# JinPLu/VeloxSeg

Measured on AMD Instinct MI355X. Metric: training patches/s on 128^3 2-mod volumes (fwd+loss+bwd+allreduce+AdamW), higher is better.
Workload: dtype f32

## Files before the change

include/veloxseg_hip.h:

```cpp
#ifndef VELOXSEG_HIP_H
#define VELOXSEG_HIP_H

#ifdef __cplusplus
extern "C" {
#endif

#define VX_ABI_VERSION 1

int vx_abi_version(void);
const char* vx_last_error(void);

int vx_conv3d_fwd(const float* x, const float* x2, int C1, const float* w, const float* bias, float* y,
                  int B, int Cin, int Di, int Hi, int Wi, int Cout, int K, int S, int P, int G, int ps, void* stream);
int vx_conv3d_bwd_data(const float* dy, const float* w, const float* bias_like, float* dx, float* dx2, int C1,
                       int B, int Cin, int Di, int Hi, int Wi, int Cout, int K, int S, int P, int G, int ps,
                       int accumulate, void* stream);
int vx_conv3d_bwd_weight(const float* x, const float* x2, int C1, const float* dy, float* dw, float* db,
                         int B, int Cin, int Di, int Hi, int Wi, int Cout, int K, int S, int P, int G, int ps, void* stream);

int vx_conv3d_bwd_weight_tiled(const float* x, const float* x2, int C1, const float* dy, float* dw, float* db,
                               int B, int Cin, int Di, int Hi, int Wi, int Cout, int K, int S, int P, int G, int ps, void* stream);
int vx_down_wgrad_ws_floats(int B, int Cin, int Di, int Hi, int Wi, int Cout);
int vx_down_wgrad_mfma(const float* x, const float* dy, float* dw, float* db, float* ws, long ws_floats,
                       int B, int Cin, int Di, int Hi, int Wi, int Cout, void* stream);
// ... 152 lines not shown
int vx_ln_cf_bwd(const float* x, const float* gamma, const float* dout, float* dx, float* dgamma, float* dbeta, float* ws,
                 int B, int C, long V, float eps, void* stream);
int vx_ln_cf_bwd_add(const float* x, const float* gamma, const float* dout, const float* add, float* dx, float* dgamma, float* dbeta, float* ws,
                     int B, int C, long V, float eps, void* stream);
int vx_ln_cf_bwd_data(const float* x, const float* gamma, const float* dout, const float* add, float* dx, float* ws, int B, int C, long V, float eps, void* stream);
int vx_ln_cf_bwd_param(const float* x, const float* dout, const float* ws, float* dgamma, float* dbeta, int B, int C, long V, void* stream);

int vx_gelu_drop_fwd(const float* a, float* h, long n, const void* seed_ptr, unsigned long long dstream, float p, void* stream);
int vx_gelu_drop_bwd(const float* dh, const float* a, float* da, long n, const void* seed_ptr, unsigned long long dstream, float p, void* stream);
int vx_axpy_drop_fwd(const float* x, const float* z, float* out, float alpha, long n, const void* seed_ptr, unsigned long long dstream, float p, void* stream);
int vx_axpy_drop_bwd(const float* dout, float* dx, float* dz, float alpha, long n, const void* seed_ptr, unsigned long long dstream, float p, void* stream);
int vx_add(const float* a, const float* b, const float* c, float* out, long n, void* stream);
int vx_add_many(const float* const* a, const float* const* b, const float* const* c, float* const* out, const long* n, int count, void* stream);
int vx_channel_sum(const float* dy, float* db, int B, int C, long V, void* stream);
int vx_space_to_depth2(const float* x, float* out, int B, int C, int Dc, int Hc, int Wc, int inverse, void* stream);
int vx_patchify(const float* x, float* out, int B, int C, int d, int h, int w, int K, void* stream);
int vx_patchify_bs(const float* x, long batch_stride, float* out, int B, int C, int d, int h, int w, int K, void* stream);
int vx_patchify_bs_h(const float* x, long batch_stride, void* out, int B, int C, int d, int h, int w, int K, int out_h16, void* stream);
int vx_patch_embed_ok(int Cin, int Cout, int Do, int Ho, int Wo, int K);
int vx_patch_embed_fwd(const float* x, long batch_stride, const float* w, const float* bias, float* y, int B, int Cin, int Cout, int Do, int Ho, int Wo, void* stream);
int vx_patch_embed_bwd_weight(const float* x, long batch_stride, const float* dy, float* dw, float* db, int B, int Cin, int Cout, int Do, int Ho, int Wo, void* stream);

typedef struct VxPwaPlan {
    int grid[3];
    int n[3];
    int heads, nb;
    int small[4][3];
    int nwin[4][3];
    int woff[4];
    int Ntot;
    int l;
} VxPwaPlan;

int vx_pwa_gather_fwd(const float* src, float* tok, const VxPwaPlan* plan, int c, int m, int M, int B, void* stream);
int vx_pwa_gather_bwd(const float* src, const float* dtok, float* dsrc, const VxPwaPlan* plan, int c, int m, int M, int B, void* stream);
int vx_pwa_gather_all_fwd(const float* const* srcs, float* tq, float* tk, float* tv, int* iq, int* ik, int* iv,
                          const VxPwaPlan* plan, int cq, int cv, int M, int B, void* stream);
int vx_pwa_gather_all_bwd(const float* dtq, const float* dtk, const float* dtv, const int* iq, const int* ik, const int* iv, float* const* dsrcs,
                          const VxPwaPlan* plan, int cq, int cv, int M, int B, void* stream);
int vx_pwa_scatter_fwd(const float* tok, float* out, const VxPwaPlan* plan, int c, int m, int M, int B, void* stream);
int vx_pwa_scatter_bwd(const float* dout, float* dtok, const VxPwaPlan* plan, int c, int m, int M, int B, void* stream);
int vx_pwa_scatter_fwd_all(const float* tok, float* const* outs, const VxPwaPlan* plan, int c, int M, int B, void* stream);
int vx_pwa_scatter_bwd_all(const float* const* douts, float* dtok, const VxPwaPlan* plan, int c, int M, int B, void* stream);
int vx_pwa_scatter_bwd_all_w(const float* const* douts, float* dtok, const VxPwaPlan* plan, int c, int M, int B, void* stream);
int vx_pwa_scatter_bwd_all_wz(const float* const* douts, float* dtok, const VxPwaPlan* plan, int c, int M, int B, float* extra_zero, long extra_floats, void* stream);
int vx_pwa_attn_set_fused_bwd(int on);
int vx_pwa_scatter_set_ident(int on);
int vx_pwa_attn_fwd(const float* Q, const float* K, const float* V, const float* table, float* O, float* LSE,
                    const VxPwaPlan* plan, int B, int M, int cq, int cv,
                    const void* seed_ptr, unsigned long long dstream, float p_drop, void* stream);
int vx_pwa_attn_bwd_ws_floats(const VxPwaPlan* plan, int B, int M);
int vx_pwa_attn_bwd_rep_offset(const VxPwaPlan* plan, int B, int M);
int vx_pwa_attn_bwd_mark_rep_zeroed(const float* delta_ws);
int vx_pwa_gather_set_vec(int on);
int vx_pwa_attn_bwd(const float* Q, const float* K, const float* V, const float* table, const float* O, const float* LSE,
                    const float* dO, float* dQ, float* dK, float* dV, float* dtable, float* delta_ws,
                    const VxPwaPlan* plan, int B, int M, int cq, int cv,
                    const void* seed_ptr, unsigned long long dstream, float p_drop, void* stream);
int vx_pwa_attn_bwd_nofold(const float* Q, const float* K, const float* V, const float* table, const float* O, const float* LSE,
                           const float* dO, float* dQ, float* dK, float* dV, float* delta_ws,
                           const VxPwaPlan* plan, int B, int M, int cq, int cv,
                           const void* seed_ptr, unsigned long long dstream, float p_drop, void* stream);
int vx_pwa_attn_bwd_fold(const float* delta_ws, float* dtable, const VxPwaPlan* plan, int B, int M, void* stream);
int vx_pwa_attn_bwd_fold_many(const float* const* delta_ws, float* const* dtables, const VxPwaPlan* const* plans, int count, int B, int M, void* stream);
int vx_pwa_attn_set_split(int S);
int vx_pwa_attn_bwd1_ok(const VxPwaPlan* plan, int B, int M, int cq, int cv);
int vx_pwa_attn_mbits_words(const VxPwaPlan* plan, int B, int M);
int vx_pwa_attn_mbits_useful(const VxPwaPlan* plan, int B, int M, int cq, int cv);
int vx_pwa_attn_set_valu_bits(int on);
int vx_pwa_attn_fwd_mb(const float* q, const float* k, const float* v, const float* table, float* out, float* lse, const VxPwaPlan* plan, int B, int M, int cq, int cv,
                       const void* seed_ptr, unsigned long long dstream, float p_drop, void* mbits, void* stream);
int vx_pwa_attn_bwd_mb(const float* q, const float* k, const float* v, const float* table, const float* out, const float* lse, const float* dout,
                       float* dq, float* dk, float* dv, float* dtable, float* delta_ws, const VxPwaPlan* plan, int B, int M, int cq, int cv,
                       const void* seed_ptr, unsigned long long dstream, float p_drop, const void* mbits, void* stream);
int vx_pwa_attn_bwd_nofold_mb(const float* q, const float* k, const float* v, const float* table, const float* out, const float* lse, const float* dout,
                              float* dq, float* dk, float* dv, float* delta_ws, const VxPwaPlan* plan, int B, int M, int cq, int cv,
                              const void* seed_ptr, unsigned long long dstream, float p_drop, const void* mbits, void* stream);
int vx_pwa_attn_mfma_ok(const VxPwaPlan* plan, int B, int M, int cq, int cv);
int vx_pwa_attn_set_mfma(int on);
int vx_pwa_attn_bwd1h_ok(const VxPwaPlan* plan, int B, int M, int cq, int cv);
int vx_pwa_attn_set_f16_bwd(int on);
int vx_pwa_attn_set_f16_bwd_ragged(int on);
int vx_pwa_attn_set_f16_bwd_m1(int on);
int vx_pwa_attn_set_short(int on);

int vx_seg_loss_fwd(const float* l0, const float* l1, const float* l2, const float* l3, int nh, const void* labels, int lab_kind,
                    double* acc, int B, int C, long V, void* stream);
int vx_sqdiff_sum(const float* a, const float* b, long n, double* acc, void* stream);
int vx_sqdiff_sum_bs(const float* a, const float* b, long n_per_sample, long b_batch_stride, int B, double* acc, void* stream);
int vx_mse_bwd_bs(const float* a, const float* b, long n_per_sample, long b_batch_stride, int B, const float* coef, const float* gout, float* da, void* stream);
int vx_sqdiff_sum_grad_bs(const float* a, const float* b, long n_per_sample, long b_batch_stride, int B, double* acc, float scale, float* da, void* stream);
int vx_sqdiff_sum_grad_bs_h(const void* a, const float* b, long n_per_sample, long b_batch_stride, int B, double* acc, float scale, void* da, int a_h16, void* stream);
int vx_loss_finalize(const double* seg_acc, int nh, int B, int C, long V, const float* head_weights,
                     const double* rc_acc, long n_rc, float w_rc,
                     const float* gram_seg, const float* g0, const float* g1, const float* g2, const float* g3, int M, int Cg, float w_f,
                     float* loss_out, float* coef, void* stream);
int vx_seg_loss_bwd(const float* logits, const void* labels, int lab_kind, const float* coef_head, const float* gout,
                    float* dlogits, int B, int C, long V, void* stream);
int vx_seg_loss_bwd4(const float* lg0, const float* lg1, const float* lg2, const float* lg3, int nh, const void* labels, int lab_kind, const float* coef,
                     int coef_stride, const float* gout, float* dl0, float* dl1, float* dl2, float* dl3, int B, int C, long V, void* stream);
int vx_seg_loss_ds_ok(int C, int D, int H, int W);
int vx_seg_loss_ds_set_columns(int on);
int vx_seg_loss_ds_ws_floats(const int* low_dims, int nh, int B, int C, int D);
int vx_seg_loss_ds_fwd(const float* l0, const float* l1, const float* l2, const float* l3, const int* low_dims, int nh, const void* labels, int lab_kind,
                       double* acc, int B, int C, int D, int H, int W, void* stream);
int vx_seg_loss_ds_bwd(const float* l0, const float* l1, const float* l2, const float* l3, const int* low_dims, int nh, const void* labels, int lab_kind,
                       const float* coef, int coef_stride, const float* gout, float* dl0, float* dl1, float* dl2, float* dl3, float* ws,
                       int B, int C, int D, int H, int W, void* stream);
int vx_seg_loss_ds_h16_ok(const int* low_dims, int nh, int B, int C, int D, int H, int W);
int vx_seg_loss_ds_fwd_h(const void* l0, const float* l1, const float* l2, const float* l3, const int* low_dims, int nh, const void* labels, int lab_kind,
                         double* acc, int B, int C, int D, int H, int W, int l0_h16, void* stream);
int vx_seg_loss_ds_bwd_h(const void* l0, const float* l1, const float* l2, const float* l3, const int* low_dims, int nh, const void* labels, int lab_kind,
                         const float* coef, int coef_stride, const float* gout, void* dl0, float* dl1, float* dl2, float* dl3, float* ws,
                         int B, int C, int D, int H, int W, int l0_h16, void* stream);
int vx_mse_bwd(const float* a, const float* b, const float* coef, const float* gout, float* da, long n, void* stream);
int vx_gram_mse_bwd(const float* gs, const float* g0, const float* g1, const float* g2, const float* g3, int M, const float* coef,
                    const float* gout, float* dgs, float* d0, float* d1, float* d2, float* d3, long n, void* stream);
int vx_gram_fwd(const float* x, float* G, int B, int C, long V, void* stream);
int vx_gram_bwd(const float* x, const float* dG, float* dx, int B, int C, long V, void* stream);
int vx_upsample_trilinear_fwd(const float* x, float* out, long BC, int d, int h, int w, int D, int H, int W, void* stream);
int vx_upsample_trilinear_bwd(const float* dout, float* dx, float* ws, long BC, int d, int h, int w, int D, int H, int W, void* stream);

int vx_upconv_set_mfma4(int on);
int vx_upconv_k2s2_fwd(const float* x, const float* w, const float* bias, float* y, int B, int Ci, int Co, int d, int h, int wd, void* stream);
int vx_upconv_k2s2_bwd_data(const float* dy, const float* w, float* dx, int B, int Ci, int Co, int d, int h, int wd, void* stream);
int vx_upconv_k2s2_wgrad_ok(int Ci, int Co);
int vx_upconv_k2s2_wgrad(const float* x, const float* dy, float* dw, int B, int Ci, int Co, int d, int h, int wd, void* stream);

int vx_adamw_step(float* p, const float* g, float* m, float* v, long n, float lr, float beta1, float beta2, float eps,
                  float weight_decay, long step, float grad_scale, void* stream);

int vx_sw_extract(const float* vol, float* win, int C, int D, int H, int W, int rd, int rh, int rw, int z0, int y0, int x0, void* stream);
int vx_sw_accumulate(const float* win, float* acc, int C, int D, int H, int W, int rd, int rh, int rw, int z0, int y0, int x0, float weight, void* stream);
int vx_sw_finalize(const float* acc, float* out, unsigned char* labels, const float* cz, const float* cy, const float* cx,
                   int C, int D, int H, int W, void* stream);
int vx_argmax_channels(const float* logits, unsigned char* labels, int B, int C, long V, void* stream);
int vx_confusion(const void* pred, int pred_bytes, const void* gt, int gt_bytes, unsigned long long* conf, int B, long V, int NC, void* stream);

int vx_min_value(const float* x, long n, float* out_init_inf, void* stream);
int vx_bbox_gt(const float* x, float thr, int C, int D, int H, int W, int* out6, void* stream);
int vx_label_chunk_count(const void* labels, int lab_bytes, long n, int chunk, int fg, int* counts, void* stream);
int vx_label_kth_in_chunk(const void* labels, int lab_bytes, long n, long chunk_start, int chunk, int fg, int k, long* out_index, void* stream);
int vx_rotate_z(const float* x, float* out, int C, int D, int H, int W, float cos_a, float sin_a, int mode, void* stream);

int vx_conv_mfma_ok(int Cin, int Cout, int D, int H, int W, int K, int S, int P, int G, int ps);
int vx_conv_mfma_set_stem_f16(int on);
int vx_conv_mfma_set_stem_pieces(int np);
int vx_conv_mfma_stem_pieces(void);
int vx_conv_mfma_ws_floats(int Cin, int Cout, int K, int backward);
int vx_conv_mfma_fwd(const float* x, const float* w, const float* bias, float* y, float* ws, int B, int Cin, int D, int H, int W, int Cout, int K, int S, int P,
                     void* stream);
int vx_conv_mfma_fwd_writes_absmax(int Cin, int Cout, int D, int H, int W, int K, int S, int P);
int vx_conv_mfma_fwd_mx(const float* x, const float* w, const float* bias, float* y, float* ws, unsigned* x_absmax, int B, int Cin, int D, int H, int W, int Cout,
                        int K, int S, int P, void* stream);
int vx_conv_mfma_bwd_data(const float* dy, const float* w, float* dx, float* ws, int B, int Cin, int D, int H, int W, int Cout, int K, int S, int P, int accumulate,
                          void* stream);

int vx_expand_split_ws_floats(int Cc, int ns);
int vx_expand_fwd_mfma_split(const float* x, const float* w, const float* bias, float* wt_ws, float* y, int B, int Cc, int D, int H, int W, int ns, void* stream);
int vx_expand_bwd_data_mfma_split(const float* dy_fine, const float* w, float* wt_ws, float* dx, int B, int Cc, int D, int H, int W, int accumulate, int ns, void* stream);
int vx_expand_split_ew_offset(int Cc);
int vx_expand_prep_split22(const float* w, float* wt_fwd, float* wt_bwd, int Cc, void* stream);
int vx_expand_fwd_mfma_split_prepared(const float* x, const float* bias, const float* wt_fwd, float* y, int B, int Cc, int D, int H, int W, void* stream);
int vx_expand_bwd_data_mfma_split_prepared(const float* dy_fine, const float* wt_bwd, const float* ew_fwd, float* dx, int B, int Cc, int D, int H, int W, int accumulate, void* stream);
int vx_expand_bwd_data_mfma_split_ew(const float* dy_fine, const float* w, float* wt_ws, float* dx, int B, int Cc, int D, int H, int W, int accumulate, int ns,
                                     const float* ew_fwd, void* stream);
// ... 55 lines not shown
```

veloxseg_amd/csrc/pwa_mfma.hip:

```cpp
#include "vx_common.h"
#include <stdlib.h>
#include "../../include/veloxseg_hip.h"

typedef float vx_f32x4 __attribute__((ext_vector_type(4)));
#define VX_MFMA(a, b, c) __builtin_amdgcn_mfma_f32_16x16x4f32((a), (b), (c), 0, 0, 0)
#define VX_DTABLE_REPLICAS 16

struct VxAttnM {
    int BH, heads, Nt, ML, l, M;
    int n[3];
    float scale;
    int lin_cst, Tsz;
    int xcd;
};

__device__ __forceinline__ void vx_am_tables(const VxAttnM& A, const float* __restrict__ table, int a, int* lin, float* bias, int nthr) {
    for (int t = threadIdx.x; t < A.l; t += nthr) {
        const int t2 = t % A.n[2], t1 = (t / A.n[2]) % A.n[1], t0 = t / (A.n[2] * A.n[1]);
        lin[t] = (t0 * (2 * A.n[1] - 1) + t1) * (2 * A.n[2] - 1) + t2;
    }
    for (int k0 = threadIdx.x; k0 < A.Tsz; k0 += nthr * 8) {
        float v[8];
#pragma unroll
        for (int u = 0; u < 8; ++u) { const int k = k0 + u * nthr; v[u] = table[(long)(k < A.Tsz ? k : 0) * A.heads + a]; }
#pragma unroll
        for (int u = 0; u < 8; ++u) { const int k = k0 + u * nthr; if (k < A.Tsz) bias[k] = v[u]; }
    }
}
template <int C>
__device__ __forceinline__ void vx_am_stage_op(float* __restrict__ dst, const float* __restrict__ src, int ML, float mul, int nthr) {
    const int n4 = ML * (C / 4);
    for (int e0 = threadIdx.x; e0 < n4; e0 += nthr * 8) {
        float4 v[8];
#pragma unroll
        for (int u = 0; u < 8; ++u) { const int e = e0 + u * nthr; v[u] = reinterpret_cast<const float4*>(src)[e < n4 ? e : 0]; }
#pragma unroll
        for (int u = 0; u < 8; ++u) {
            const int e = e0 + u * nthr;
            if (e < n4) {
                const int row = e / (C / 4), ks = e - row * (C / 4);
                float* d = dst + ((row >> 4) * (C / 4) + ks) * 64 + (row & 15);
                d[0] = v[u].x * mul; d[16] = v[u].y * mul; d[32] = v[u].z * mul; d[48] = v[u].w * mul;
            }
        }
    }
}
template <int C> __device__ __forceinline__ int vx_am_op_index(int tile, int r, int c) { return ((tile * (C / 4) + (c >> 2)) * 64) + (c & 3) * 16 + r; }

template <int CQ, int CV>
__global__ void __launch_bounds__(512) vx_pwa_attn_mfma_fwd_k(const float* __restrict__ Q, const float* __restrict__ K, const float* __restrict__ Vt,
                                                              const float* __restrict__ table, float* __restrict__ O, float* __restrict__ LSE,
                                                              VxAttnM A, VxDrop drop, unsigned short* __restrict__ mbits) {
    constexpr int KSQ = CQ / 4, CVB = (CV + 15) / 16, SV = CV + 1;
    extern __shared__ __attribute__((aligned(16))) float vx_am_lds[];
    int* __restrict__ lin = reinterpret_cast<int*>(vx_am_lds);
    float* __restrict__ bias = vx_am_lds + ((A.l + 3) & ~3);
    float* __restrict__ Kop = bias + ((A.Tsz + 3) & ~3);
    float* __restrict__ Vs = Kop + A.ML * CQ;
    int bx_, by_;
    vx_xcd_rows(bx_, by_, A.xcd & 1);
    const long win = by_;
    const int a = (int)((win / A.Nt) % A.heads);
    const float* __restrict__ kp = K + win * A.ML * CQ;
    const float* __restrict__ vp = Vt + win * A.ML * CV;
    vx_am_tables(A, table, a, lin, bias, 512);
    {
        const int n4 = A.ML * KSQ;
        for (int e0 = threadIdx.x; e0 < n4; e0 += 512 * 8) {
            float4 v[8];
#pragma unroll
            for (int u = 0; u < 8; ++u) { const int e = e0 + u * 512; v[u] = reinterpret_cast<const float4*>(kp)[e < n4 ? e : 0]; }
#pragma unroll
            for (int u = 0; u < 8; ++u) {
                const int e = e0 + u * 512;
                if (e < n4) {
                    const int key = e / KSQ, ks = e - key * KSQ;
                    const int it = key >> 6, w = key & 63, tu = (w >> 2) & 3, mrow = 4 * (w >> 4) + (w & 3);
                    float* d = Kop + ((4 * it + tu) * KSQ + ks) * 64 + mrow;
                    d[0] = v[u].x; d[16] = v[u].y; d[32] = v[u].z; d[48] = v[u].w;
                }
            }
        }
    }
    for (int e0 = threadIdx.x; e0 < A.ML * (CV / 4); e0 += 512 * 8) {
        float4 v[8];
#pragma unroll
        for (int u = 0; u < 8; ++u) { const int e = e0 + u * 512; v[u] = reinterpret_cast<const float4*>(vp)[e < A.ML * (CV / 4) ? e : 0]; }
#pragma unroll
        for (int u = 0; u < 8; ++u) {
            const int e = e0 + u * 512;
            if (e < A.ML * (CV / 4)) { const int key = e / (CV / 4), c4 = e - key * (CV / 4); float* d = Vs + key * SV + 4 * c4; d[0] = v[u].x; d[1] = v[u].y; d[2] = v[u].z; d[3] = v[u].w; }
        }
    }
    __syncthreads();
    const int lane = threadIdx.x & 63, wave = threadIdx.x >> 6, m = lane & 15, qg = lane >> 4;
    const int q0 = (bx_ * 8 + wave) * 16;
    if (q0 >= A.ML) return;
    const VxDropCtx dc = vx_attn_ctx(drop);
    const long row = win * A.ML + q0 + m;
    float qb[KSQ];
#pragma unroll
    for (int ks = 0; ks < KSQ; ++ks) qb[ks] = Q[row * CQ + 4 * ks + qg] * A.scale;
    const int lin_q = lin[(q0 + m) % A.l] + A.lin_cst;
    float mrun = -INFINITY, lsum = 0.0f;
    vx_f32x4 oacc[CVB];
#pragma unroll
    for (int cb = 0; cb < CVB; ++cb) oacc[cb] = (vx_f32x4){0.f, 0.f, 0.f, 0.f};
    constexpr int KU = 4;
    const int ntile = A.ML / 16;
    vx_f32x4 oacc2[CVB];
#pragma unroll
    for (int cb = 0; cb < CVB; ++cb) oacc2[cb] = (vx_f32x4){0.f, 0.f, 0.f, 0.f};
    for (int kt0 = 0; kt0 < ntile; kt0 += KU) {
        vx_f32x4 s[KU];
        int4 lk[KU];
#pragma unroll
        for (int u = 0; u < KU; ++u) {
            s[u] = (vx_f32x4){0.f, 0.f, 0.f, 0.f};
            lk[u] = *reinterpret_cast<const int4*>(&lin[(16 * (kt0 + qg)) % A.l + 4 * u]);
        }
#pragma unroll
        for (int ks = 0; ks < KSQ; ++ks)
#pragma unroll
            for (int u = 0; u < KU; ++u) s[u] = VX_MFMA(Kop[((kt0 + u) * KSQ + ks) * 64 + lane], qb[ks], s[u]);
        float mt = -INFINITY;
#pragma unroll
        for (int u = 0; u < KU; ++u) {
            s[u][0] += bias[lin_q - lk[u].x]; s[u][1] += bias[lin_q - lk[u].y]; s[u][2] += bias[lin_q - lk[u].z]; s[u][3] += bias[lin_q - lk[u].w];
            mt = fmaxf(mt, fmaxf(fmaxf(s[u][0], s[u][1]), fmaxf(s[u][2], s[u][3])));
        }
        mt = fmaxf(mt, __shfl_xor(mt, 16, 64));
        mt = fmaxf(mt, __shfl_xor(mt, 32, 64));
        const float mn = fmaxf(mrun, mt);
        const float alpha = __expf(mrun - mn);
        mrun = mn;
// ... 889 lines not shown
                    o4.x += dqT[0]; o4.y += dqT[1]; o4.z += dqT[2]; o4.w += dqT[3];
                    *dst = o4;
                }
            }
            {
                const _Float16* tcol = tq + m * VX_BH_TS + 16 * j + 4 * qg;
                const uint2 q0 = *reinterpret_cast<const uint2*>(tcol), q1 = *reinterpret_cast<const uint2*>(tcol + nq);
                const uint2 o0 = *reinterpret_cast<const uint2*>(tcol + 16 * VX_BH_TS), o1 = *reinterpret_cast<const uint2*>(tcol + 16 * VX_BH_TS + nq);
                const vx_au4 aQ = {q0.x, q0.y, q1.x, q1.y}, aO = {o0.x, o0.y, o1.x, o1.y};
#pragma unroll
                for (int f = 0; f < MF; ++f) {
                    dv[f] = VX_MFMA_H(aO, ((vx_au4){pmh[f][0], pmh[f][1], pmh[f][2], pmh[f][3]}), dv[f]);
                    dv[f] = VX_MFMA_H(aO, ((vx_au4){pml[f][0], pml[f][1], pml[f][2], pml[f][3]}), dv[f]);
                    dk[f] = VX_MFMA_H(aQ, ((vx_au4){dsh[f][0], dsh[f][1], dsh[f][2], dsh[f][3]}), dk[f]);
                    dk[f] = VX_MFMA_H(aQ, ((vx_au4){dsl[f][0], dsl[f][1], dsl[f][2], dsl[f][3]}), dk[f]);
                }
            }
#pragma unroll
            for (int i = 0; i < 4; ++i) { if (kval) gw[raw[i] - wbase] += dssum[i]; __builtin_amdgcn_wave_barrier(); }
        }
        const float fK = A.scale * ldexpf(1.0f, -(eq + ed + ev)), fV = ldexpf(1.0f, -ed), fQ = A.scale * ldexpf(1.0f, -(ek + ed + ev)), fB = ldexpf(1.0f, -(ed + ev));
#pragma unroll
        for (int f = 0; f < MF; ++f)
#pragma unroll
            for (int i = 0; i < 4; ++i) { totk[f][i] = fmaf(dk[f][i], fK, totk[f][i]); totv[f][i] = fmaf(dv[f][i], fV, totv[f][i]); }
        __syncthreads();
        constexpr int img = NR * C;
        for (int e = threadIdx.x; e < img; e += 256) {
            const int c = e % C, r2 = e / C, f = r2 / nq, t = 16 * q_lo + (r2 - f * nq);
            float* dst = dQ + (wrow + (long)f * A.l + t) * C + c;
            const float v = ((dqw[e] + dqw[img + e]) + (dqw[2 * img + e] + dqw[3 * img + e])) * fQ;
            dqw[e] = 0.0f; dqw[img + e] = 0.0f; dqw[2 * img + e] = 0.0f; dqw[3 * img + e] = 0.0f;
            if ((RAG && t >= A.l) || f >= MF) continue;
            if (atomic_dq) atomicAdd(dst, v); else *dst = v;
        }
        {
            const int* wb_s = reinterpret_cast<const int*>(red) + 16;
            constexpr int NU = RAG ? 4 : 2;
            float gsum[NU];
#pragma unroll
            for (int u = 0; u < NU; ++u) {
                const int x = threadIdx.x + 256 * u;
                float g = 0.0f;
                if (x < 2 * WIN) {
#pragma unroll
                    for (int w = 0; w < 4; ++w) {
                        const int y = x - wb_s[w];
                        if (y >= 0 && y < WIN) g += (gwin[(4 * w) * WIN + y] + gwin[(4 * w + 1) * WIN + y]) + (gwin[(4 * w + 2) * WIN + y] + gwin[(4 * w + 3) * WIN + y]);
                    }
                }
                gsum[u] = g;
            }
            __syncthreads();
#pragma unroll
            for (int u = 0; u < NU; ++u) {
                const int x = threadIdx.x + 256 * u;
                const int k = bbase + x + A.lin_cst;
                if (gsum[u] != 0.0f && k >= 0 && k < A.Tsz) atomicAdd(dtab_dst + (long)k * A.heads + a, gsum[u] * fB);
            }
            for (int e = threadIdx.x; e < 16 * WIN; e += 256) gwin[e] = 0.0f;
        }
    }
#pragma unroll
    for (int f = 0; f < MF; ++f) {
        const long kr = wrow + (long)f * A.l + kcc;
        float k4[4], v4[4];
#pragma unroll
        for (int i = 0; i < 4; ++i) {
            k4[i] = totk[f][i] + __shfl_xor(totk[f][i], 4 * C, 64);
            v4[i] = totv[f][i] + __shfl_xor(totv[f][i], 4 * C, 64);
        }
        if (4 * qg < C && kval) {
            if (QS == 1) {
                *reinterpret_cast<float4*>(dK + kr * C + 4 * qg) = make_float4(k4[0], k4[1], k4[2], k4[3]);
                *reinterpret_cast<float4*>(dV + kr * C + 4 * qg) = make_float4(v4[0], v4[1], v4[2], v4[3]);
            } else {
#pragma unroll
                for (int i = 0; i < 4; ++i) { atomicAdd(dK + kr * C + 4 * qg + i, k4[i]); atomicAdd(dV + kr * C + 4 * qg + i, v4[i]); }
            }
        }
    }
}

static bool vx_am_fill(VxAttnM& A, const VxPwaPlan* P, int B, int M, int cq) {
    A.BH = B * P->heads; A.heads = P->heads; A.Nt = P->Ntot; A.l = P->l; A.M = M; A.ML = M * P->l;
    A.n[0] = P->n[0]; A.n[1] = P->n[1]; A.n[2] = P->n[2];
    A.scale = 1.0f / sqrtf((float)cq);
    A.lin_cst = ((P->n[0] - 1) * (2 * P->n[1] - 1) + (P->n[1] - 1)) * (2 * P->n[2] - 1) + (P->n[2] - 1);
    A.Tsz = (2 * A.n[0] - 1) * (2 * A.n[1] - 1) * (2 * A.n[2] - 1);
    A.xcd = 3;
    return true;
}
static size_t vx_am_tab_floats(const VxAttnM& A) { return (size_t)((A.l + 3) & ~3) + (size_t)((A.Tsz + 3) & ~3); }
static size_t vx_am_lds_fwd(const VxAttnM& A, int cq, int cv) { return (vx_am_tab_floats(A) + (size_t)A.ML * cq + (size_t)A.ML * (cv + 2)) * 4; }
static size_t vx_am_lds_q(const VxAttnM& A, int cq, int cv) { return (vx_am_tab_floats(A) + (size_t)4 * ((A.Tsz + 3) & ~3) + (size_t)A.ML * (cq + cv)) * 4; }
static size_t vx_am_lds_kv(const VxAttnM& A, int cq, int cv) { return (vx_am_tab_floats(A) + (size_t)A.ML * (cq + cv + 2)) * 4; }

static int vx_am_enabled = 3;
extern "C" int vx_pwa_attn_set_mfma(int mask) { vx_am_enabled = mask & 15; return 0; }

extern "C" int vx_pwa_attn_mfma_ok(const VxPwaPlan* P, int B, int M, int cq, int cv) {
    const int want = (vx_am_enabled & 1) | ((vx_am_enabled & 4) ? 2 : 0);
    if (!want || P == nullptr || B <= 0 || M <= 0) return 0;
    if (P->l % 64 != 0 || cq % 4 != 0 || cq > 16 || cv % 4 != 0 || cv > 32) return 0;
    if (!((cq == 4 && cv == 4) || (cq == 8 && cv == 8) || (cq == 8 && cv == 16) || (cq == 16 && cv == 32) || (cq == 16 && cv == 16) || (cq == 4 && cv == 8))) return 0;
    VxAttnM A;
    vx_am_fill(A, P, B, M, cq);
    const size_t cap = 150 * 1024;
    return (vx_am_lds_fwd(A, cq, cv) <= cap && vx_am_lds_q(A, cq, cv) <= cap && vx_am_lds_kv(A, cq, cv) <= cap) ? want : 0;
}

template <int A_, int B_> struct vx_am_pair { static constexpr int a = A_, b = B_; };
template <class F> static bool vx_am_dispatch(int cq, int cv, F&& f) {
#define VX_CASE(X, Y) if (cq == X && cv == Y) { f(vx_am_pair<X, Y>{}); return true; }
    VX_CASE(4, 4) VX_CASE(8, 8) VX_CASE(8, 16) VX_CASE(16, 32) VX_CASE(16, 16) VX_CASE(4, 8)
#undef VX_CASE
    return false;
}
template <class K> static void vx_am_attr(K kernel) { (void)hipFuncSetAttribute((const void*)kernel, hipFuncAttributeMaxDynamicSharedMemorySize, 160 * 1024); }

int vx_pwa_attn_mfma_fwd(const float* Q, const float* K, const float* V, const float* table, float* O, float* LSE, unsigned short* mbits, const VxPwaPlan* plan, int B, int M,
                         int cq, int cv, VxDrop d, void* stream) {
    VxAttnM A;
    vx_am_fill(A, plan, B, M, cq);
    const dim3 grid(vx_cdiv(A.ML / 16, 8), (unsigned)((long)A.BH * A.Nt));
    const size_t shm = vx_am_lds_fwd(A, cq, cv);
    vx_am_dispatch(cq, cv, [&](auto pr) {
        constexpr int CQ = decltype(pr)::a, CV = decltype(pr)::b;
        static bool once = false;
        if (!once) { vx_am_attr(vx_pwa_attn_mfma_fwd_k<CQ, CV>); once = true; }
        vx_pwa_attn_mfma_fwd_k<CQ, CV><<<grid, dim3(512), shm, (hipStream_t)stream>>>(Q, K, V, table, O, LSE, A, d, mbits);
    });
    return 0;
}
int vx_pwa_attn_mfma_bwd(const float* Q, const float* K, const float* V, const float* table, const float* O, const float* LSE, const float* dO, float* dQ,
                         float* dK, float* dV, float* dtable, float* delta, float* rep, const VxPwaPlan* plan, int B, int M, int cq, int cv, VxDrop d,
                         void* stream) {
    VxAttnM A;
    vx_am_fill(A, plan, B, M, cq);
    const dim3 grid(vx_cdiv(A.ML / 16, 8), (unsigned)((long)A.BH * A.Nt));
    const size_t shm_q = vx_am_lds_q(A, cq, cv), shm_kv = vx_am_lds_kv(A, cq, cv);
    vx_am_dispatch(cq, cv, [&](auto pr) {
        constexpr int CQ = decltype(pr)::a, CV = decltype(pr)::b;
        static bool once = false;
        if (!once) { vx_am_attr(vx_pwa_attn_mfma_bwd_q_k<CQ, CV>); vx_am_attr(vx_pwa_attn_mfma_bwd_kv_k<CQ, CV>); once = true; }
        vx_pwa_attn_mfma_bwd_q_k<CQ, CV><<<grid, dim3(512), shm_q, (hipStream_t)stream>>>(Q, K, V, table, O, LSE, dO, dQ, delta, rep, A, d);
        vx_pwa_attn_mfma_bwd_kv_k<CQ, CV><<<grid, dim3(512), shm_kv, (hipStream_t)stream>>>(Q, K, V, table, LSE, delta, dO, dK, dV, rep, dtable, A, d);
    });
    return 0;
}

struct VxB1Geo { int NT, waves_used, nbx, QS, NTq, win; size_t shm; };
static int vx_b1_span(const VxAttnM& A, int ntok, int step) {
    int worst = 0;
    for (int t0 = 0; t0 < A.l; t0 += step) {
        int lo = 1 << 30, hi = -(1 << 30);
        for (int t = t0; t < t0 + ntok; ++t) {
            const int tc = t < A.l ? t : A.l - 1;
            const int t2 = tc % A.n[2], t1 = (tc / A.n[2]) % A.n[1], tz = tc / (A.n[2] * A.n[1]);
            const int v = (tz * (2 * A.n[1] - 1) + t1) * (2 * A.n[2] - 1) + t2;
            lo = v < lo ? v : lo; hi = v > hi ? v : hi;
        }
        worst = (hi - lo) > worst ? (hi - lo) : worst;
    }
    return worst;
}
static VxB1Geo vx_b1_geo(const VxAttnM& A, int cq, int mf, bool few_windows = false) {
    VxB1Geo g;
    g.NT = (A.l + 15) / 16;
    g.waves_used = g.NT < 4 ? g.NT : 4;
    g.nbx = (g.NT + g.waves_used - 1) / g.waves_used;
    g.NTq = g.NT < 4 ? g.NT : 4;
    if (few_windows) g.NTq = 1;
    while (g.NT % g.NTq) --g.NTq;
    g.QS = g.NT / g.NTq;
    const int sq = vx_b1_span(A, g.NTq * 16, g.NTq * 16), sk16 = vx_b1_span(A, 16, 16), sk64 = vx_b1_span(A, 16 * g.waves_used, 16 * g.waves_used);
    g.win = (sq + sk16 + 1 <= VX_B1_WIN && sq + sk64 + 1 <= 2 * VX_B1_WIN) ? 1 : 0;
    const size_t lp = (size_t)g.NT * 16, nq = (size_t)g.NTq * 16, tpad = (size_t)((A.Tsz + 3) & ~3);
    g.shm = (lp + (g.win ? 2 * VX_B1_WIN + 4 * VX_B1_WIN : 2 * tpad) + 2 * mf * nq + 4 * mf * nq * cq + (size_t)4 * mf * 16 * 20) * sizeof(float);
    return g;
}
struct VxZeroMany { float4* p[4]; long n4[4]; };
__global__ void __launch_bounds__(256) vx_zero_many_k(VxZeroMany z) {
    float4* __restrict__ p = z.p[blockIdx.y];
    const long n = z.n4[blockIdx.y];
#pragma unroll
    for (int u = 0; u < 4; ++u) {
        const long i = ((long)blockIdx.x * 4 + u) * 256 + threadIdx.x;
        if (i < n) p[i] = make_float4(0.f, 0.f, 0.f, 0.f);
    }
}
static bool vx_b1_short(const VxAttnM& A) { return A.M == 1 && A.l < 512; }
static int g_b1_short = 1;
static int vx_b1_short_on() { return g_b1_short; }
extern "C" int vx_pwa_attn_set_short(int on) { g_b1_short = on ? 1 : 0; return 0; }
static bool vx_b1_few(const VxAttnM& A) {
    const int NT = (A.l + 15) / 16;
    const bool use = vx_b1_short_on() && vx_b1_short(A) && A.l % 16 == 0;
    return use && NT >= 2 && (long)A.BH * A.Nt * ((NT + 3) / 4) * ((NT + 3) / 4) < 64;
}
extern "C" int vx_pwa_attn_bwd1_ok(const VxPwaPlan* P, int B, int M, int cq, int cv) {
    if (!(vx_am_enabled & 10) || (vx_am_enabled & 4) || P == nullptr || B <= 0 || M < 1 || M > 2) return 0;
    if (!((cq == 4 && cv == 4) || (cq == 8 && cv == 8) || (cq == 8 && cv == 16) || (cq == 16 && cv == 32) || (cq == 16 && cv == 16) || (cq == 4 && cv == 8))) return 0;
    VxAttnM A;
    vx_am_fill(A, P, B, M, cq);
    const bool prefer = (vx_am_enabled & 8) || P->l % 16 != 0 || vx_b1_few(A) || (vx_b1_short_on() && vx_b1_short(A));
    if (!prefer) return 0;
    return vx_b1_geo(A, cq, M, vx_b1_few(A)).shm <= 80 * 1024 ? 1 : 0;
}
int vx_pwa_attn_bwd1(const float* Q, const float* K, const float* V, const float* table, const float* O, const float* LSE, const float* dO, float* dQ,
                     float* dK, float* dV, float* rep, const unsigned short* mbits, const VxPwaPlan* plan, int B, int M, int cq, int cv, VxDrop d, void* stream) {
    VxAttnM A;
    vx_am_fill(A, plan, B, M, cq);
    const long nwin = (long)A.BH * A.Nt;
// ... 120 lines not shown
```

Baseline: 1089.

## Add f16 split-precision MFMA forward path for paired-window attention

Adds a new forward kernel for equal head widths 4 and 8 that splits K, V, Q and the probabilities into f16 hi/lo pairs with per-window power-of-two scaling, then runs f16 MFMA in place of the f32 16x16x4 MFMA. Softmax moves to the exp2 domain with the bias table pre-scaled by log2e and a lazy max rescale threshold. K and V are packed into a more compact LDS image, which lowers shared-memory use. The new path is on by default and carries accuracy risk from the split-f16 approximation and the thresholded max update.

Measured after the change: 1093 (median of 6 runs). No clear change (+0.3%).

```diff
diff --git a/include/veloxseg_hip.h b/include/veloxseg_hip.h
--- a/include/veloxseg_hip.h
+++ b/include/veloxseg_hip.h
@@ -258,6 +258,7 @@
 int vx_pwa_attn_set_f16_bwd(int on);
 int vx_pwa_attn_set_f16_bwd_ragged(int on);
 int vx_pwa_attn_set_f16_bwd_m1(int on);
+int vx_pwa_attn_set_f16_fwd(int on);
 int vx_pwa_attn_set_short(int on);
 
 int vx_seg_loss_fwd(const float* l0, const float* l1, const float* l2, const float* l3, int nh, const void* labels, int lab_kind,
diff --git a/veloxseg_amd/csrc/pwa_mfma.hip b/veloxseg_amd/csrc/pwa_mfma.hip
--- a/veloxseg_amd/csrc/pwa_mfma.hip
+++ b/veloxseg_amd/csrc/pwa_mfma.hip
@@ -14,7 +14,7 @@
     int xcd;
 };
 
-__device__ __forceinline__ void vx_am_tables(const VxAttnM& A, const float* __restrict__ table, int a, int* lin, float* bias, int nthr) {
+__device__ __forceinline__ void vx_am_tables(const VxAttnM& A, const float* __restrict__ table, int a, int* lin, float* bias, int nthr, float mul = 1.0f) {
     for (int t = threadIdx.x; t < A.l; t += nthr) {
         const int t2 = t % A.n[2], t1 = (t / A.n[2]) % A.n[1], t0 = t / (A.n[2] * A.n[1]);
         lin[t] = (t0 * (2 * A.n[1] - 1) + t1) * (2 * A.n[2] - 1) + t2;
@@ -24,7 +24,7 @@
 #pragma unroll
         for (int u = 0; u < 8; ++u) { const int k = k0 + u * nthr; v[u] = table[(long)(k < A.Tsz ? k : 0) * A.heads + a]; }
 #pragma unroll
-        for (int u = 0; u < 8; ++u) { const int k = k0 + u * nthr; if (k < A.Tsz) bias[k] = v[u]; }
+        for (int u = 0; u < 8; ++u) { const int k = k0 + u * nthr; if (k < A.Tsz) bias[k] = v[u] * mul; }
     }
 }
 template <int C>
@@ -48,9 +48,9 @@
 template <int C> __device__ __forceinline__ int vx_am_op_index(int tile, int r, int c) { return ((tile * (C / 4) + (c >> 2)) * 64) + (c & 3) * 16 + r; }
 
 template <int CQ, int CV>
-__global__ void __launch_bounds__(512) vx_pwa_attn_mfma_fwd_k(const float* __restrict__ Q, const float* __restrict__ K, const float* __restrict__ Vt,
-                                                              const float* __restrict__ table, float* __restrict__ O, float* __restrict__ LSE,
-                                                              VxAttnM A, VxDrop drop, unsigned short* __restrict__ mbits) {
+__device__ __forceinline__ void vx_am_fwd_f32(const float* __restrict__ Q, const float* __restrict__ K, const float* __restrict__ Vt,
+                                              const float* __restrict__ table, float* __restrict__ O, float* __restrict__ LSE,
+                                              const VxAttnM& A, const VxDrop& drop, unsigned short* __restrict__ mbits) {
     constexpr int KSQ = CQ / 4, CVB = (CV + 15) / 16, SV = CV + 1;
     extern __shared__ __attribute__((aligned(16))) float vx_am_lds[];
     int* __restrict__ lin = reinterpret_cast<int*>(vx_am_lds);
@@ -1106,6 +1106,221 @@
     }
 }
 
+__device__ __forceinline__ uint32_t vx_attn_keep16(const VxDropCtx& c, uint64_t idx0) {
+    uint32_t w = 0;
+#pragma unroll
+    for (int h = 0; h < 2; ++h) {
+        uint32_t r[4];
+        vx_philox4(c.seed, c.stream, (idx0 >> 3) + h, r);
+#pragma unroll
+        for (int x = 0; x < 4; ++x) {
+            w |= ((r[x] & 0xffffu) >= c.thr16 ? 1u : 0u) << (8 * h + 2 * x);
+            w |= ((r[x] >> 16) >= c.thr16 ? 1u : 0u) << (8 * h + 2 * x + 1);
+        }
+    }
+    return w;
+}
+#define VX_FH_PEXP 12.0f
+template <int C, bool DROP>
+__device__ __forceinline__ void vx_am_fwd_h(const float* __restrict__ Q, const float* __restrict__ K, const float* __restrict__ Vt,
+                                            const float* __restrict__ table, float* __restrict__ O, float* __restrict__ LSE,
+                                            const VxAttnM& A, const VxDrop& drop, unsigned short* __restrict__ mbits) {
+    static_assert(C == 4 || C == 8, "head widths (4, 4) and (8, 8)");
+    constexpr int C2 = C / 2, KT = C == 8 ? 32 : 16, VR = 2 * C;
+    constexpr float LOG2E = 1.4426950408889634f, LN2 = 0.6931471805599453f;
+    extern __shared__ __attribute__((aligned(16))) float vx_am_lds[];
+    int* __restrict__ lin = reinterpret_cast<int*>(vx_am_lds);
+    float* __restrict__ bias = vx_am_lds + ((A.l + 3) & ~3);
+    float* __restrict__ red = bias + ((A.Tsz + 3) & ~3);
+    vx_au4* __restrict__ Kimg = reinterpret_cast<vx_au4*>(red + 16);
+    vx_au4* __restrict__ Vimg = Kimg + (A.ML >> 4) * KT;
+    int bx_, by_;
+    vx_xcd_rows(bx_, by_, A.xcd & 1);
+    const long win = by_;
+    const int a = (int)((win / A.Nt) % A.heads);
+    const float4* __restrict__ kp4 = reinterpret_cast<const float4*>(K + win * A.ML * C);
+    const float4* __restrict__ vp4 = reinterpret_cast<const float4*>(Vt + win * A.ML * C);
+    const int lane = threadIdx.x & 63, wave = threadIdx.x >> 6, m = lane & 15, qg = lane >> 4;
+    const int npair = A.ML >> 1;
+    auto load_pair = [&](int e, float (&kk)[2 * C], float (&vv)[2 * C]) {
+#pragma unroll
+        for (int x = 0; x < C2; ++x) {
+            const float4 k4 = kp4[e * C2 + x], v4 = vp4[e * C2 + x];
+            kk[4 * x] = k4.x; kk[4 * x + 1] = k4.y; kk[4 * x + 2] = k4.z; kk[4 * x + 3] = k4.w;
+            vv[4 * x] = v4.x; vv[4 * x + 1] = v4.y; vv[4 * x + 2] = v4.z; vv[4 * x + 3] = v4.w;
+        }
+    };
+    auto max_pair = [&](const float (&kk)[2 * C], const float (&vv)[2 * C], float& km, float& vm) {
+#pragma unroll
+        for (int x = 0; x < 2 * C; ++x) { km = fmaxf(km, fabsf(kk[x])); vm = fmaxf(vm, fabsf(vv[x])); }
+    };
+    const bool own = (int)threadIdx.x < npair;
+    float k0[2 * C], v0[2 * C];
+    load_pair(own ? (int)threadIdx.x : 0, k0, v0);
+    vx_am_tables(A, table, a, lin, bias, 512, LOG2E);
+    float kmax = 0.0f, vmax = 0.0f;
+    if (own) max_pair(k0, v0, kmax, vmax);
+    for (int e = threadIdx.x + 512; e < npair; e += 512) {
+        float k1[2 * C], v1[2 * C];
+        load_pair(e, k1, v1);
+        max_pair(k1, v1, kmax, vmax);
+    }
+    kmax = vx_wave_max(kmax); vmax = vx_wave_max(vmax);
+    if (lane == 0) { red[wave] = kmax; red[8 + wave] = vmax; }
+    for (int t = threadIdx.x; t < A.l; t += 512) lin[t] *= 4;
+    __syncthreads();
+    kmax = fmaxf(fmaxf(fmaxf(red[0], red[1]), fmaxf(red[2], red[3])), fmaxf(fmaxf(red[4], red[5]), fmaxf(red[6], red[7])));
+    vmax = fmaxf(fmaxf(fmaxf(red[8], red[9]), fmaxf(red[10], red[11])), fmaxf(fmaxf(red[12], red[13]), fmaxf(red[14], red[15])));
+    const int ek = vx_a_exp(kmax, 10), ev = vx_a_exp(vmax, 8);
+    const float sk = ldexpf(1.0f, ek), sv = ldexpf(1.0f, ev);
+    auto put_pair = [&](int e, const float (&kk)[2 * C], const float (&vv)[2 * C]) {
+#pragma unroll
+        for (int j = 0; j < 2; ++j) {
+            const int key = 2 * e + j, w = key & 63, tile = 4 * (key >> 6) + ((w >> 2) & 3), mrow = 4 * (w >> 4) + (w & 3);
+            uint32_t h[C2], l[C2];
+#pragma unroll
+            for (int x = 0; x < C2; ++x) vx_a_split2(kk[j * C + 2 * x] * sk, kk[j * C + 2 * x + 1] * sk, h[x], l[x]);
+            if constexpr (C == 8) {
+                Kimg[tile * KT + mrow] = (vx_au4){h[0], h[1], h[2], h[3]};
+                Kimg[tile * KT + 16 + mrow] = (vx_au4){l[0], l[1], l[2], l[3]};
+            } else Kimg[tile * KT + mrow] = (vx_au4){h[0], h[1], l[0], l[1]};
+        }
+        {
+            const int key = 2 * e, w = key & 63, blk = (2 * (key >> 6) + ((w >> 3) & 1)) * 4 + (w >> 4), rot = C == 8 ? blk : (blk >> 1);
+            uint32_t* __restrict__ vw = reinterpret_cast<uint32_t*>(Vimg + blk * VR) + ((w & 7) >> 1);
+#pragma unroll
+            for (int c = 0; c < C; ++c) {
+                uint32_t h, l;
+                vx_a_split2(vv[c] * sv, vv[C + c] * sv, h, l);
+                vw[4 * ((c + rot) & (VR - 1))] = h;
+                vw[4 * ((C + c + rot) & (VR - 1))] = l;
+            }
+        }
+    };
+    if (own) put_pair(threadIdx.x, k0, v0);
+    for (int e = threadIdx.x + 512; e < npair; e += 512) {
+        float k1[2 * C], v1[2 * C];
+        load_pair(e, k1, v1);
+        put_pair(e, k1, v1);
+    }
+    __syncthreads();
+    const int q0 = (bx_ * 8 + wave) * 16;
+    if (q0 >= A.ML) return;
+    VxDropCtx dc;
+    if constexpr (DROP) dc = vx_attn_ctx(drop);
+    const long row = win * A.ML + q0 + m;
+    vx_au4 qB;
+    float cS;
+    {
+        float qv[C], qmax = 0.0f;
+#pragma unroll
+        for (int x = 0; x < C / 4; ++x) {
+            const float4 q4 = *reinterpret_cast<const float4*>(Q + row * C + 4 * x);
+            qv[4 * x] = q4.x; qv[4 * x + 1] = q4.y; qv[4 * x + 2] = q4.z; qv[4 * x + 3] = q4.w;
+        }
+#pragma unroll
+        for (int x = 0; x < C; ++x) qmax = fmaxf(qmax, fabsf(qv[x]));
+        qmax = vx_wave_max(qmax);
+        const int eq = vx_a_exp(qmax, 10);
+        const float sq = ldexpf(1.0f, eq);
+        uint32_t h[C2], l[C2];
+#pragma unroll
+        for (int x = 0; x < C2; ++x) vx_a_split2(qv[2 * x] * sq, qv[2 * x + 1] * sq, h[x], l[x]);
+        if constexpr (C == 8) {
+            const bool lo_ = (qg & 1) != 0;
+            qB = (vx_au4){lo_ ? l[0] : h[0], lo_ ? l[1] : h[1], lo_ ? l[2] : h[2], lo_ ? l[3] : h[3]};
+        } else {
+            qB = qg == 0 ? (vx_au4){h[0], h[1], h[0], h[1]} : (qg == 1 ? (vx_au4){l[0], l[1], l[0], l[1]} : (vx_au4){0u, 0u, 0u, 0u});
+        }
+        cS = A.scale * LOG2E * ldexpf(1.0f, -(ek + eq));
+    }
+    const char* __restrict__ bias_q = reinterpret_cast<const char*>(bias) + (lin[(q0 + m) % A.l] + 4 * A.lin_cst);
+    const vx_au4* __restrict__ kA = Kimg + (C == 8 ? (qg >> 1) * 16 : 0) + m;
+    const int vrow = m & (VR - 1);
+    float mrun = -INFINITY, lsum = 0.0f;
+    vx_f32x4 oa = {0.f, 0.f, 0.f, 0.f}, ob = {0.f, 0.f, 0.f, 0.f};
+    const int ntrip = A.ML >> 6;
+    int koff = 16 * qg;
+    for (int it = 0; it < ntrip; ++it) {
+        vx_au4 ka[4], va[2];
+        int4 lk[4];
+#pragma unroll
+        for (int u = 0; u < 4; ++u) ka[u] = kA[(4 * it + u) * KT];
+#pragma unroll
+        for (int u = 0; u < 4; ++u) lk[u] = *reinterpret_cast<const int4*>(&lin[koff + 4 * u]);
+#pragma unroll
+        for (int hh = 0; hh < 2; ++hh) {
+            const int blk = (2 * it + hh) * 4 + qg, rot = C == 8 ? blk : (blk >> 1);
+            va[hh] = Vimg[blk * VR + ((vrow + rot) & (VR - 1))];
+        }
+        koff += 64;
+        if (koff >= A.l) koff -= A.l;
+        vx_f32x4 s[4];
+#pragma unroll
+        for (int u = 0; u < 4; ++u) s[u] = VX_MFMA_H(ka[u], qB, ((vx_f32x4){0.f, 0.f, 0.f, 0.f}));
+        uint32_t kw = 0xffffu;
+        if constexpr (DROP) {
+            kw = vx_attn_keep16(dc, (uint64_t)row * (uint64_t)A.ML + (uint64_t)(64 * it + 16 * qg));
+            if (mbits != nullptr) mbits[(win * (A.ML >> 4) + (4 * it + qg)) * A.ML + q0 + m] = (unsigned short)kw;
+        }
+        auto bq = [&](int off) { return *reinterpret_cast<const float*>(bias_q - off); };
+        vx_af2 t[8];
+        const vx_af2 cS2 = {cS, cS};
+#pragma unroll
+        for (int u = 0; u < 4; ++u) {
+            t[2 * u] = (vx_af2){s[u][0], s[u][1]} * cS2 + (vx_af2){bq(lk[u].x), bq(lk[u].y)};
+            t[2 * u + 1] = (vx_af2){s[u][2], s[u][3]} * cS2 + (vx_af2){bq(lk[u].z), bq(lk[u].w)};
+        }
+        float mt = fmaxf(t[0][0], t[0][1]);
+#pragma unroll
+        for (int x = 1; x < 8; ++x) mt = fmaxf(mt, fmaxf(t[x][0], t[x][1]));
+        mt = fmaxf(mt, __shfl_xor(mt, 16, 64));
+        mt = fmaxf(mt, __shfl_xor(mt, 32, 64));
+        const float mn = fmaxf(mrun, mt - VX_FH_PEXP);
+        const float alpha = __builtin_amdgcn_exp2f(mrun - mn);
+        mrun = mn;
+        const vx_af2 mn2 = {mn, mn};
+        vx_af2 ps2 = {0.f, 0.f};
+        uint32_t ph[8], pl[8];
+#pragma unroll
+        for (int x = 0; x < 8; ++x) {
+            const vx_af2 d = t[x] - mn2;
+            vx_af2 p = {__builtin_amdgcn_exp2f(d[0]), __builtin_amdgcn_exp2f(d[1])};
+            ps2 += p;
+            if constexpr (DROP) { p[0] = ((kw >> (2 * x)) & 1u) ? p[0] : 0.0f; p[1] = ((kw >> (2 * x + 1)) & 1u) ? p[1] : 0.0f; }
+            vx_a_split2(p[0], p[1], ph[x], pl[x]);
+        }
+        const float psum = ps2[0] + ps2[1];
+        lsum = lsum * alpha + psum;
+        oa *= alpha; ob *= alpha;
+        oa = VX_MFMA_H(va[0], ((vx_au4){ph[0], ph[1], ph[2], ph[3]}), oa);
+        ob = VX_MFMA_H(va[1], ((vx_au4){ph[4], ph[5], ph[6], ph[7]}), ob);
+        oa = VX_MFMA_H(va[0], ((vx_au4){pl[0], pl[1], pl[2], pl[3]}), oa);
+        ob = VX_MFMA_H(va[1], ((vx_au4){pl[4], pl[5], pl[6], pl[7]}), ob);
+    }
+    oa += ob;
+    float o[4];
+#pragma unroll
+    for (int i = 0; i < 4; ++i) o[i] = oa[i] + __shfl_xor(oa[i], C == 8 ? 32 : 16, 64);
+    lsum += __shfl_xor(lsum, 16, 64);
+    lsum += __shfl_xor(lsum, 32, 64);
+    float inv = ldexpf(1.0f, -ev) / lsum;
+    if constexpr (DROP) inv *= dc.inv_keep;
+    if (qg < C / 4) *reinterpret_cast<float4*>(O + row * C + 4 * qg) = make_float4(o[0] * inv, o[1] * inv, o[2] * inv, o[3] * inv);
+    if (qg == 0) LSE[row] = fmaf(mrun, LN2, __log2f(lsum) * LN2);
+}
+
+template <int CQ, int CV, int PIPE>
+__global__ void __launch_bounds__(512) vx_pwa_attn_mfma_fwd_k(const float* __restrict__ Q, const float* __restrict__ K, const float* __restrict__ Vt,
+                                                              const float* __restrict__ table, float* __restrict__ O, float* __restrict__ LSE,
+                                                              VxAttnM A, VxDrop drop, unsigned short* __restrict__ mbits) {
+    if constexpr (PIPE == 0) vx_am_fwd_f32<CQ, CV>(Q, K, Vt, table, O, LSE, A, drop, mbits);
+    else {
+        static_assert(CQ == CV, "the f16-pipe forward: equal head widths");
+        vx_am_fwd_h<CQ, PIPE == 2>(Q, K, Vt, table, O, LSE, A, drop, mbits);
+    }
+}
+
 static bool vx_am_fill(VxAttnM& A, const VxPwaPlan* P, int B, int M, int cq) {
     A.BH = B * P->heads; A.heads = P->heads; A.Nt = P->Ntot; A.l = P->l; A.M = M; A.ML = M * P->l;
     A.n[0] = P->n[0]; A.n[1] = P->n[1]; A.n[2] = P->n[2];
@@ -1117,6 +1332,7 @@
 }
 static size_t vx_am_tab_floats(const VxAttnM& A) { return (size_t)((A.l + 3) & ~3) + (size_t)((A.Tsz + 3) & ~3); }
 static size_t vx_am_lds_fwd(const VxAttnM& A, int cq, int cv) { return (vx_am_tab_floats(A) + (size_t)A.ML * cq + (size_t)A.ML * (cv + 2)) * 4; }
+static size_t vx_am_lds_fwd_h(const VxAttnM& A, int c) { return (vx_am_tab_floats(A) + 16) * 4 + (size_t)A.ML * 8 * c; }
 static size_t vx_am_lds_q(const VxAttnM& A, int cq, int cv) { return (vx_am_tab_floats(A) + (size_t)4 * ((A.Tsz + 3) & ~3) + (size_t)A.ML * (cq + cv)) * 4; }
 static size_t vx_am_lds_kv(const VxAttnM& A, int cq, int cv) { return (vx_am_tab_floats(A) + (size_t)A.ML * (cq + cv + 2)) * 4; }
 
@@ -1141,6 +1357,8 @@
 #undef VX_CASE
     return false;
 }
+static int vx_am_f16_fwd = 1;
+extern "C" int vx_pwa_attn_set_f16_fwd(int on) { vx_am_f16_fwd = on ? 1 : 0; return 0; }
 template <class K> static void vx_am_attr(K kernel) { (void)hipFuncSetAttribute((const void*)kernel, hipFuncAttributeMaxDynamicSharedMemorySize, 160 * 1024); }
 
 int vx_pwa_attn_mfma_fwd(const float* Q, const float* K, const float* V, const float* table, float* O, float* LSE, unsigned short* mbits, const VxPwaPlan* plan, int B, int M,
@@ -1148,12 +1366,24 @@
     VxAttnM A;
     vx_am_fill(A, plan, B, M, cq);
     const dim3 grid(vx_cdiv(A.ML / 16, 8), (unsigned)((long)A.BH * A.Nt));
+    if (vx_am_f16_fwd && cq == cv && (cq == 4 || cq == 8)) {
+        const size_t shm = vx_am_lds_fwd_h(A, cq);
+        const bool dropping = d.seed_ptr != nullptr && d.p > 0.0f;
+        static bool once[4] = {false, false, false, false};
+        auto go = [&](auto kernel, int slot) {
+            if (!once[slot]) { vx_am_attr(kernel); once[slot] = true; }
+            kernel<<<grid, dim3(512), shm, (hipStream_t)stream>>>(Q, K, V, table, O, LSE, A, d, mbits);
+        };
+        if (cq == 4) { if (dropping) go(vx_pwa_attn_mfma_fwd_k<4, 4, 2>, 0); else go(vx_pwa_attn_mfma_fwd_k<4, 4, 1>, 1); }
+        else { if (dropping) go(vx_pwa_attn_mfma_fwd_k<8, 8, 2>, 2); else go(vx_pwa_attn_mfma_fwd_k<8, 8, 1>, 3); }
+        return 0;
+    }
     const size_t shm = vx_am_lds_fwd(A, cq, cv);
     vx_am_dispatch(cq, cv, [&](auto pr) {
         constexpr int CQ = decltype(pr)::a, CV = decltype(pr)::b;
         static bool once = false;
-        if (!once) { vx_am_attr(vx_pwa_attn_mfma_fwd_k<CQ, CV>); once = true; }
-        vx_pwa_attn_mfma_fwd_k<CQ, CV><<<grid, dim3(512), shm, (hipStream_t)stream>>>(Q, K, V, table, O, LSE, A, d, mbits);
+        if (!once) { vx_am_attr(vx_pwa_attn_mfma_fwd_k<CQ, CV, 0>); once = true; }
+        vx_pwa_attn_mfma_fwd_k<CQ, CV, 0><<<grid, dim3(512), shm, (hipStream_t)stream>>>(Q, K, V, table, O, LSE, A, d, mbits);
     });
     return 0;
 }
```
